# donglinb/ORB-SLAM-BIRDVIEW

Hardware: AMD Instinct MI355X
Metric: ORB features/sec per GPU (1280×720, 2000 kp, 8 levels) + Hamming matches/sec (higher is better)
Workload: dtype u8; 1 GPU; C3 1280x720 KITTI-style synthetic, 2000 features, 8 levels; width=1280, height=720, nfeatures=2000, nlevels=8, ini_th_fast=20, min_th_fast=7, batch_per_gpu=256, global_batch=256, parallelism=frame-sharded x1 (no collective), batches_in_flight=2

## Files before the change

### orb-slam-birdview_amd/csrc/extract_kernels.hip

```cpp
#include "glibc_trig.h"
#include "orbgpu_internal.h"
#include "pattern31_data.inc"

#include <algorithm>
#include <cstring>

namespace orbgpu {

__constant__ __attribute__((aligned(16))) int8_t c_pattern[1024] = {ORBGPU_PATTERN31_VALUES};
__constant__ __attribute__((aligned(16))) float c_pattern_f[1024] = {ORBGPU_PATTERN31_VALUES};

struct IcMaskTable {
    uint32_t m[64][4];
};
constexpr IcMaskTable make_ic_masks() {
    IcMaskTable t{};
    constexpr int umax[16] = {15, 15, 15, 15, 14, 14, 14, 13, 13, 12, 11, 10, 9, 8, 6, 3};
    for (int l = 0; l < 64; l++) {
        const int r = (l >> 1) < 30 ? (l >> 1) : 30, v = r - 15, h = l & 1;
        const int d = umax[v < 0 ? -v : v];
        for (int i = 0; i < 4; i++) {
            uint32_t m = 0;
            for (int j = 0; j < 4; j++) {
                const int u = 4 * (4 * h + i) + j;
                if (u >= 15 - d && u <= 15 + d) m |= 0xFFu << (8 * j);
            }
            t.m[l][i] = m;
        }
    }
    return t;
}
__constant__ __attribute__((aligned(16))) IcMaskTable c_ic_masks = make_ic_masks();

namespace {

struct LevelPtr {
    const uint8_t* p;
    int stride;
};

__device__ __forceinline__ LevelPtr level_ptr(const Geom* __restrict__ g, int l, const uint8_t* frames,
                                              long long framePitch, int rowStride, const uint8_t* pyr, int f) {
    if (l == 0) return {frames + (long long)f * framePitch, rowStride};
    return {pyr + (long long)f * g->pyr_bytes + g->L[l].pyr_off, g->L[l].pitch};
}

__device__ __forceinline__ void wave_lds_sync() {
    __builtin_amdgcn_fence(__ATOMIC_RELEASE, "wavefront");
    __builtin_amdgcn_wave_barrier();
    __builtin_amdgcn_fence(__ATOMIC_ACQUIRE, "wavefront");
}

__device__ __forceinline__ int lanes_below(unsigned long long mask) {
    return __builtin_amdgcn_mbcnt_hi((unsigned)(mask >> 32), __builtin_amdgcn_mbcnt_lo((unsigned)mask, 0));
}

}

typedef unsigned short ushort2_t __attribute__((ext_vector_type(2)));

__device__ __forceinline__ unsigned mul_hi_u24(unsigned a, unsigned b) {
    unsigned r;
    asm("v_mul_hi_u32_u24 %0, %1, %2" : "=v"(r) : "v"(a), "v"(b));
    return r;
}
typedef unsigned int uint32x4_t __attribute__((ext_vector_type(4)));

template <bool GENERIC>
__global__ __launch_bounds__(256) void k_resize(const Geom* __restrict__ g, const ResizeCoef* __restrict__ coef,
                                                int level, const uint8_t* __restrict__ frames, long long framePitch,
                                                int rowStride, uint8_t* __restrict__ pyr) {
    const int f = blockIdx.z;
    const int dw = g->L[level].w, dh = g->L[level].h;
    const int x0 = (blockIdx.x * 64 + (threadIdx.x & 63)) * 4;
    const int y = blockIdx.y * 4 + (threadIdx.x >> 6);
    if (x0 >= dw || y >= dh) return;
    const LevelPtr src = level_ptr(g, level - 1, frames, framePitch, rowStride, pyr, f);
    const ResizeCoef cy = coef[dw + y];
    const uint8_t* r0 = src.p + (long long)cy.s0 * src.stride;
    const uint8_t* r1 = src.p + (long long)cy.s1 * src.stride;
    uint32_t packed = 0;
#pragma unroll
    for (int i = 0; i < 4; i++) {
        const int x = min(x0 + i, dw - 1);
        const ResizeCoef cx = coef[x];
        const unsigned h0 = __umul24(r0[cx.s0], (unsigned)cx.c0) + __umul24(r0[cx.s1], (unsigned)cx.c1);
        const unsigned h1 = __umul24(r1[cx.s0], (unsigned)cx.c0) + __umul24(r1[cx.s1], (unsigned)cx.c1);
        const unsigned v =
            GENERIC ? min((__umul24((unsigned)cy.c0, h0) + __umul24((unsigned)cy.c1, h1) + (1u << 21)) >> 22, 255u)
                    : ((__umul24((unsigned)cy.c0, h0 >> 4) >> 16) + (__umul24((unsigned)cy.c1, h1 >> 4) >> 16) + 2) >> 2;
        packed |= (uint32_t)v << (8 * i);
    }
    uint8_t* dst = pyr + (long long)f * g->pyr_bytes + g->L[level].pyr_off;
    *reinterpret_cast<uint32_t*>(dst + (long long)y * g->L[level].pitch + x0) = packed;
}

template <bool GENERIC>
__device__ __forceinline__ int4 rs_row_entry(const ResizeCoef& c, int sy0) {
    return make_int4(__mul24(c.s0 - sy0, kRsPitch), __mul24(c.s1 - sy0, kRsPitch), GENERIC ? c.c0 : c.c0 << 12,
                     GENERIC ? c.c1 : c.c1 << 12);
}
template <bool GENERIC>
__device__ __forceinline__ unsigned rs_vpass(unsigned c0, unsigned c1, unsigned h0, unsigned h1) {
    if (GENERIC) return min((__umul24(c0, h0) + __umul24(c1, h1) + (1u << 21)) >> 22, 255u);
    return (mul_hi_u24(c0, h0 & ~15u) + mul_hi_u24(c1, h1 & ~15u) + 2) >> 2;
}

constexpr int kCpSc1 = 16;

__constant__ unsigned kRsMagic[18] = {0,    65536, 32768, 21846, 16384, 13108, 10923, 9363, 8192,
                                      7282, 6554,  5958,  5462,  5042,  4682,  4370,  4096, 3856};
template <int kRsTileH, bool GENERIC, int CP, int KP = 0>
__device__ __forceinline__ void resize_tile(const Geom* __restrict__ g, const ResizeCoef* __restrict__ coef, int level,
                                            const uint8_t* __restrict__ frames, long long framePitch, int rowStride,
                                            uint8_t* __restrict__ pyr, int f, int bx, int by, int tid, uint8_t* s_src,
                                            int4* s_cx, int4* s_cy, bool active) {
    constexpr int kRows = rs_rows(kRsTileH);
    constexpr int kQ = kRsPitch / 16;
    constexpr int kPer = KP > 0 ? KP : (kRows * kQ + 255) / 256;
    const int dw = g->L[level].w, dh = g->L[level].h;
    const int x0 = bx * kRsTileW, y0 = by * kRsTileH;
    const LevelPtr src = level_ptr(g, level - 1, frames, framePitch, rowStride, pyr, f);
    const int nx = min(kRsTileW, dw - x0), ny = min(kRsTileH, dh - y0);
    if (!active) {
        __syncthreads();
        return;
    }
    const bool vec16 = ((reinterpret_cast<uintptr_t>(src.p) | (uintptr_t)src.stride) & 15) == 0;
    const int sx0 = coef[x0].s0 & (vec16 ? ~15 : ~3), sx1 = coef[x0 + nx - 1].s1;
    const int sy0 = coef[dw + y0].s0, sy1 = coef[dw + y0 + ny - 1].s1;
    const int nr = sy1 - sy0 + 1;
    const uint8_t* base = src.p + (long long)sy0 * src.stride + sx0;
    int4 cxv = make_int4(0, 0, 0, 0), cyv = make_int4(0, 0, 0, 0);
    if (vec16) {
        const int nq = ((sx1 - sx0) >> 4) + 1;
        const unsigned magic = kRsMagic[nq];
        const int total = nr * nq;
        const uint64_t pb = reinterpret_cast<uint64_t>(base);
        const auto rsrc = __builtin_amdgcn_make_buffer_rsrc(reinterpret_cast<void*>(pb), 0, 0x7FFFFFFF, 0x00020000);
        uint4 v[kPer];
#pragma unroll
        for (int k = 0; k < kPer; k++) {
            const int i = min(tid + 256 * k, total - 1);
            const int r = (int)(__umul24((unsigned)i, magic) >> 16), q = i - (int)__umul24((unsigned)r, (unsigned)nq);
            const uint32x4_t w = __builtin_amdgcn_raw_buffer_load_b128(rsrc, (int)__umul24((unsigned)r, (unsigned)src.stride) + 16 * q, 0, CP);
            v[k] = make_uint4(w[0], w[1], w[2], w[3]);
        }
        if (tid < kRsTileW) {
            const ResizeCoef c = coef[x0 + min(tid, nx - 1)];
            cxv = make_int4(c.s0, c.s1, c.c0, c.c1);
        }
        if (tid < kRsTileH) {
            const ResizeCoef c = coef[dw + y0 + min(tid, ny - 1)];
            cyv = rs_row_entry<GENERIC>(c, sy0);
        }
#pragma unroll
        for (int k = 0; k < kPer; k++) {
            const int i = min(tid + 256 * k, total - 1);
            const int r = (int)(__umul24((unsigned)i, magic) >> 16), q = i - (int)__umul24((unsigned)r, (unsigned)nq);
            *reinterpret_cast<uint4*>(&s_src[r * kRsPitch + 16 * q]) = v[k];
        }
    } else {
        if (tid < kRsTileW) {
            const ResizeCoef c = coef[x0 + min(tid, nx - 1)];
            cxv = make_int4(c.s0, c.s1, c.c0, c.c1);
        }
        if (tid < kRsTileH) {
            const ResizeCoef c = coef[dw + y0 + min(tid, ny - 1)];
            cyv = rs_row_entry<GENERIC>(c, sy0);
        }
        if (((reinterpret_cast<uintptr_t>(src.p) | (uintptr_t)src.stride) & 3) == 0) {
            const int nw = (sx1 - sx0 + 4) >> 2;
            for (int i = tid; i < nr * 68; i += 256) {
                const int r = i / 68, wd = i - r * 68;
                if (wd < nw)
                    *reinterpret_cast<uint32_t*>(&s_src[r * kRsPitch + 4 * wd]) =
                        *reinterpret_cast<const uint32_t*>(base + (long long)r * src.stride + 4 * wd);
            }
        } else {
            const int nb = sx1 - sx0 + 1;
            for (int i = tid; i < nr * kRsPitch; i += 256) {
                const int r = i / kRsPitch, b = i - r * kRsPitch;
                if (b < nb) s_src[r * kRsPitch + b] = base[(long long)r * src.stride + b];
            }
        }
    }
    if (tid < kRsTileW) s_cx[tid] = cxv;
    if (tid < kRsTileH) s_cy[tid] = cyv;
// ... 2 lines not shown
    int o0[4], o1[4];
    unsigned c0[4], c1[4];
#pragma unroll
    for (int i = 0; i < 4; i++) {
        const int4 cx = s_cx[tx + i];
        o0[i] = cx.x - sx0;
        o1[i] = cx.y - sx0;
        c0[i] = cx.z;
        c1[i] = cx.w;
    }
    const uint64_t lb = reinterpret_cast<uint64_t>(pyr + (long long)f * g->pyr_bytes + g->L[level].pyr_off);
    const auto dsr = __builtin_amdgcn_make_buffer_rsrc(
        reinterpret_cast<void*>(((uint64_t)(uint32_t)__builtin_amdgcn_readfirstlane((unsigned)(lb >> 32)) << 32) |
                                (uint64_t)(uint32_t)__builtin_amdgcn_readfirstlane((unsigned)lb)),
        0, 0x7FFFFFFF, 0x00020000);
    const int pitch = g->L[level].pitch;
    const unsigned dcol = (unsigned)(x0 + tx);
    if (tx >= nx) return;
    const int bo = o0[0];
    const bool packed_ok = o1[3] - bo <= 7;
    if (__builtin_amdgcn_ballot_w64(!packed_ok) == 0) {
        unsigned sel[4];
        uint32_t cc[4];
#pragma unroll
        for (int i = 0; i < 4; i++) {
            sel[i] = (unsigned)(o0[i] - bo) | 0x0C00u | ((unsigned)(o1[i] - bo) << 16) | 0x0C000000u;
            cc[i] = c0[i] | (c1[i] << 16);
        }
        const int bw = bo >> 2, bsh = bo & 3;
#pragma unroll
        for (int pass = 0; pass < kRsTileH / 8; pass++) {
            const int ty = pass * 8 + (tid >> 5);
            if (ty >= ny) break;
            const int4 cy = s_cy[ty];
            const unsigned cy0 = (unsigned)cy.z, cy1 = (unsigned)cy.w;
            const uint32_t* q0 = reinterpret_cast<const uint32_t*>(&s_src[cy.x]) + bw;
            const uint32_t* q1 = reinterpret_cast<const uint32_t*>(&s_src[cy.y]) + bw;
            const uint32_t u0 = q0[0], u1 = q0[1], u2 = q0[2], w0 = q1[0], w1 = q1[1], w2 = q1[2];
            const uint32_t a0 = __builtin_amdgcn_alignbyte(u1, u0, bsh), a1 = __builtin_amdgcn_alignbyte(u2, u1, bsh);
            const uint32_t b0 = __builtin_amdgcn_alignbyte(w1, w0, bsh), b1 = __builtin_amdgcn_alignbyte(w2, w1, bsh);
            uint32_t packed = 0;
#pragma unroll
            for (int i = 0; i < 4; i++) {
                const unsigned h0 = __builtin_amdgcn_udot2(__builtin_bit_cast(ushort2_t, cc[i]),
                                                           __builtin_bit_cast(ushort2_t, __builtin_amdgcn_perm(a1, a0, sel[i])), 0u, false);
                const unsigned h1 = __builtin_amdgcn_udot2(__builtin_bit_cast(ushort2_t, cc[i]),
                                                           __builtin_bit_cast(ushort2_t, __builtin_amdgcn_perm(b1, b0, sel[i])), 0u, false);
                const unsigned v = rs_vpass<GENERIC>(cy0, cy1, h0, h1);
                packed |= v << (8 * i);
            }
            __builtin_amdgcn_raw_buffer_store_b32(packed, dsr, (int)(__umul24((unsigned)(y0 + ty), (unsigned)pitch) + dcol), 0, CP);
        }
        return;
    }
#pragma unroll
    for (int pass = 0; pass < kRsTileH / 8; pass++) {
        const int ty = pass * 8 + (tid >> 5);
        if (ty >= ny) break;
        const int4 cy = s_cy[ty];
        const uint8_t* r0 = &s_src[cy.x];
        const uint8_t* r1 = &s_src[cy.y];
        uint32_t packed = 0;
#pragma unroll
        for (int i = 0; i < 4; i++) {
            const unsigned h0 = __umul24(r0[o0[i]], c0[i]) + __umul24(r0[o1[i]], c1[i]);
            const unsigned h1 = __umul24(r1[o0[i]], c0[i]) + __umul24(r1[o1[i]], c1[i]);
            const unsigned v = rs_vpass<GENERIC>((unsigned)cy.z, (unsigned)cy.w, h0, h1);
            packed |= v << (8 * i);
        }
        __builtin_amdgcn_raw_buffer_store_b32(packed, dsr, (int)(__umul24((unsigned)(y0 + ty), (unsigned)pitch) + dcol), 0, CP);
    }
}

template <int kRsTileH, bool GENERIC, int KP>
__global__ __launch_bounds__(256) void k_resize_tiled(const Geom* __restrict__ g,
                                                      const ResizeCoef* __restrict__ coef, int level,
                                                      const uint8_t* __restrict__ frames, long long framePitch,
                                                      int rowStride, uint8_t* __restrict__ pyr) {
    extern __shared__ __attribute__((aligned(16))) uint8_t s_src[];
    __shared__ int4 s_cx[kRsTileW];
    __shared__ int4 s_cy[kRsTileH];
    resize_tile<kRsTileH, GENERIC, 0, KP>(g, coef, level, frames, framePitch, rowStride, pyr, blockIdx.z, blockIdx.x,
                                          blockIdx.y, threadIdx.x, s_src, s_cx, s_cy, true);
}

template <int CP>
__device__ __forceinline__ uint32_t chain_ld32(const uint8_t* p) {
    if constexpr (CP != 0)
        return __hip_atomic_load(reinterpret_cast<const uint32_t*>(p), __ATOMIC_RELAXED, __HIP_MEMORY_SCOPE_AGENT);
    else return *reinterpret_cast<const uint32_t*>(p);
}
template <int CP>
__device__ __forceinline__ uint32_t chain_ld8(const uint8_t* p) {
    if constexpr (CP != 0) {
        const uintptr_t a = reinterpret_cast<uintptr_t>(p);
        const uint32_t w = __hip_atomic_load(reinterpret_cast<const uint32_t*>(a & ~(uintptr_t)3), __ATOMIC_RELAXED,
                                             __HIP_MEMORY_SCOPE_AGENT);
        return (w >> (8 * (a & 3))) & 0xFFu;
    } else {
        return *p;
    }
}

template <bool GENERIC, int CP>
__device__ __forceinline__ void chain_job(const Geom* __restrict__ g, const ResizeCoef* __restrict__ coef,
                                          const ChainJob* __restrict__ J, const ChainSegment& sg, const RcoefOff& roff,
                                          const uint8_t* __restrict__ frames, long long framePitch, int rowStride,
                                          uint8_t* __restrict__ pyr, int f, int tid, uint8_t* sm, int4* sreg) {
    const int l = J->level, b = J->base;
    if (tid <= l) sreg[tid] = J->reg[tid];
    uint8_t* buf0 = sm;
    uint8_t* buf1 = sm + sg.buf_bytes;
    int4* sc = reinterpret_cast<int4*>(sm + 2 * sg.buf_bytes);
    uint8_t* fp = pyr + (long long)f * g->pyr_bytes;
    __syncthreads();
    {
        int e0 = 0;
        for (int k = b + 1; k <= l; k++) {
            const int4 R = sreg[k], S = sreg[k - 1];
            const int nx = R.y - R.x, ny = R.w - R.z;
            const int sp = (S.y - S.x + 3) & ~3;
            const ResizeCoef* cx = coef + roff.o[k];
            const int wk = g->L[k].w;
            for (int e = tid; e < nx + ny; e += 256) {
                int4 v;
                if (e < nx) {
                    const ResizeCoef c = cx[min(R.x + e, wk - 1)];
                    v = make_int4(c.s0 - S.x, c.s1 - S.x, c.c0, c.c1);
                } else {
                    const ResizeCoef c = cx[wk + R.z + (e - nx)];
                    v = rs_row_entry<GENERIC>(c, S.z);
                    v.x = (c.s0 - S.z) * sp;
                    v.y = (c.s1 - S.z) * sp;
                }
                sc[e0 + e] = v;
            }
            e0 += nx + ny;
        }
    }
    {
        const int4 R = sreg[b];
        const int p0 = (R.y - R.x + 3) & ~3, nq = p0 >> 2, ny = R.w - R.z, wb = g->L[b].w;
        const uint8_t* src = b == 0 ? frames + (long long)f * framePitch : fp + g->L[b].pyr_off;
        const int stride = b == 0 ? rowStride : g->L[b].pitch;
        const bool al = ((reinterpret_cast<uintptr_t>(src) | (uintptr_t)stride) & 3) == 0;
        const int QW = nq <= 16 ? 16 : nq <= 32 ? 32 : 64, RP = 256 / QW;
        for (int qb = 0; qb < nq; qb += QW)
            for (int r = tid / QW; r < ny; r += RP) {
                const int q = qb + (tid & (QW - 1));
                if (q >= nq) continue;
                const int col = R.x + 4 * q;
                const uint8_t* rp = src + (long long)(R.z + r) * stride;
                uint32_t v;
                if (al && col + 3 < wb) {
                    v = chain_ld32<CP>(rp + col);
                } else {
                    v = 0;
                    for (int t = 0; t < 4; t++)
                        if (col + t < wb) v |= chain_ld8<CP>(rp + col + t) << (8 * t);
                }
                *reinterpret_cast<uint32_t*>(buf0 + r * p0 + 4 * q) = v;
            }
    }
    __syncthreads();
    int e0 = 0;
    for (int k = b + 1; k <= l; k++) {
// ... 2085 lines not shown
            for (int l = 1; l < nl; l++)
                if (cseg[l] == sgi) lo = std::min(lo, l), hi = std::max(hi, l);
            for (int l = hi; l >= lo; l--) chainl(l);
            for (int l = hi; l >= lo; l--) {
                fast(l);
                octree(l);
            }
        }
    }
    for (int l = 0; l < nl; l++) {
        const int cap = g.L[l].kp_cap;
        for (int i = 0; i < cap; i += 16)
            for (int f = 0; f < nframes; f++)
                push(kFlowDescribe, l, f, -1, g.L[l].kp_base + i, std::min(16, cap - i), ctr(f, 2, 0), l + 1, 1);
    }
    constexpr int kLds = 160 * 1024 - 64;
    const int need = std::max({16 * g.fast_wave_bytes, 16 * kDescWaveBytes + 256, 4 * rsq, (int)octree_lds_bytes(g.node_cap)});
    if (need > kLds) return false;
    plan.ntasks = (int)tasks.size();
    plan.nframes = nframes;
    plan.nctr = kFlowCtrBase + 4 * nl * nframes;
    plan.lds_bytes = kLds;
    const long long room = kLds - (long long)octree_lds_bytes(g.node_cap);
    const long long want = ((long long)g.max_level_cand + 7) & ~7LL;
    plan.lds_keys = room > 0 ? (int)std::min(want, (room / 6) & ~7LL) : 0;
    plan.rs_quarter = rsq;
    plan.blocks = std::max(1, blocks);
    return true;
}

FlowArgs flow_args(const ExtractBuffers& b, const uint8_t* d_frames, long long frame_pitch, int row_stride, int nframes,
                   orb_keypoint* d_kps, uint8_t* d_desc, int* d_counts, int kp_cap) {
    FlowArgs A;
    std::memset(&A, 0, sizeof A);
    A.g = b.d_geom;
    A.rcoef = b.d_rcoef;
    std::memcpy(A.roff.o, b.rcoef_off, sizeof A.roff.o);
    A.cells = b.d_cells;
    A.frames = d_frames;
    A.framePitch = frame_pitch;
    A.rowStride = row_stride;
    A.pyr = b.d_pyr;
    A.cands = b.d_cands;
    A.candFirst = b.d_candFirst;
    A.keys = b.d_keys;
    A.knode = b.d_knode;
    A.lvlKps = b.d_lvlKps;
    A.lvlCount = b.d_lvlCount;
    A.err = b.d_err;
    A.errHost = b.err_host;
    A.outK = d_kps;
    A.outD = d_desc;
    A.outN = d_counts;
    A.kpCap = kp_cap;
    A.tasks = b.d_flow;
    A.ntasks = b.flow.ntasks;
    A.nframes = nframes;
    A.ctr = b.d_flow_ctr;
    A.ldsKeys = b.flow.lds_keys;
    A.rsQuarter = b.flow.rs_quarter;
    A.stamps = b.d_flow_stamps;
    A.chainJobs = b.d_chain;
    for (int i = 0; i < ORBGPU_MAX_LEVELS; i++) A.chainSeg[i] = b.flow_chain.seg[i];
    return A;
}

hipError_t launch_extract(const Geom& g, const ExtractBuffers& b, const uint8_t* d_frames, long long frame_pitch,
                          int row_stride, int nframes, orb_keypoint* d_kps, uint8_t* d_desc, int* d_counts,
                          int kp_cap, hipStream_t stream, KernelMarker marker, void* user) {
    if (nframes <= 0) return hipSuccess;
    if (b.d_flow && b.flow.nframes == nframes) {
        const bool fma = !(g.variant & ORB_VARIANT_NO_FMA);
        auto kern = g.fast_compact ? (fma ? k_extract_flow<48, true> : k_extract_flow<48, false>)
                                   : (fma ? k_extract_flow<kFastTilePitch, true> : k_extract_flow<kFastTilePitch, false>);
        if (marker) marker(user, ORB_K_FLOW, 1, stream);
        hipLaunchKernelGGL(kern, dim3(b.flow.blocks), dim3(kFlowThreads), (size_t)b.flow.lds_bytes, stream, b.d_flow_args);
        if (marker) marker(user, ORB_K_FLOW, 0, stream);
        return hipGetLastError();
    }
    auto resize = [&](int l, hipStream_t s) {
        const int t = g.L[l].rs_tiled;
        const ResizeCoef* cf = b.d_rcoef + b.rcoef_off[l];
        const bool gen = (g.variant & ORB_VARIANT_RESIZE_GENERIC) != 0;
        if (t & 3) {
            const int th = (t & 2) ? 32 : 16;
            const dim3 grid(cdiv(g.L[l].w, kRsTileW), cdiv(g.L[l].h, th), nframes);
            const size_t lds = (size_t)g.L[l].rs_span_rows * kRsPitch;
            const int kp = g.L[l].rs_chunks <= 512 ? 2 : g.L[l].rs_chunks <= 768 ? 3 : 0;
            auto kern = th == 32 ? (gen ? (kp == 2 ? k_resize_tiled<32, true, 2> : kp == 3 ? k_resize_tiled<32, true, 3>
                                                                                          : k_resize_tiled<32, true, 0>)
                                        : (kp == 2 ? k_resize_tiled<32, false, 2> : kp == 3 ? k_resize_tiled<32, false, 3>
                                                                                           : k_resize_tiled<32, false, 0>))
                                 : (gen ? (kp == 2 ? k_resize_tiled<16, true, 2> : k_resize_tiled<16, true, 0>)
                                        : (kp == 2 ? k_resize_tiled<16, false, 2> : k_resize_tiled<16, false, 0>));
            hipLaunchKernelGGL(kern, grid, dim3(256), lds, s, b.d_geom, cf, l, d_frames, frame_pitch, row_stride,
                               b.d_pyr);
        } else {
            hipLaunchKernelGGL(gen ? k_resize<true> : k_resize<false>, dim3(cdiv(g.L[l].w, 256), cdiv(g.L[l].h, 4), nframes),
                               dim3(256), 0, s, b.d_geom, cf, l, d_frames, frame_pitch, row_stride, b.d_pyr);
        }
    };
    auto fast = [&](int cbeg, int cnum, hipStream_t s, int* zero) {
        const int items = cnum * nframes;
        auto kern = g.fast_compact ? k_fast_wave<48> : k_fast_wave<kFastTilePitch>;
        const int ipw = nframes == 1 ? 1 : 2;
        hipLaunchKernelGGL(kern, dim3(cdiv(items, ipw)), dim3(64), (size_t)g.fast_wave_bytes, s, b.d_geom, b.d_cells,
                           d_frames, frame_pitch, row_stride, b.d_pyr, b.d_cands, b.d_candFirst, items, cbeg, cnum,
                           b.d_stamps, zero, ipw);
    };
    auto octree = [&](int lbase, int nl, hipStream_t s, int* err) {
        const bool one = nframes * nl <= 256;
        const int lk = one ? octree_lds_keys_whole_cu(g) : octree_lds_keys(g.node_cap);
        hipLaunchKernelGGL(k_octree<kOctreeThreads>, dim3(nframes, nl), dim3(kOctreeThreads),
                           octree_lds_bytes(g.node_cap) + (size_t)lk * 6, s, b.d_geom, b.d_cands, b.d_candFirst,
                           b.d_keys, b.d_knode, b.d_lvlKps, b.d_lvlCount, err, lk,
                           b.d_stamps ? b.d_stamps + (size_t)nframes * g.ncells * 8 : nullptr, lbase);
    };
    auto describe = [&](hipStream_t s) {
        unsigned long long* dst = b.d_stamps ? b.d_stamps + (size_t)nframes * (g.ncells * 8 + g.nlevels * 32) : nullptr;
        const int spw = nframes == 1 ? 1 : kDescSlotsPerWave;
        const unsigned gx = cdiv(g.nkpcap, kDescWaves * spw);
        hipLaunchKernelGGL((g.variant & ORB_VARIANT_NO_FMA) ? k_describe<false> : k_describe<true>, dim3(gx * nframes), dim3(64 * kDescWaves), 0, s, b.d_geom, d_frames, frame_pitch,
                           row_stride, b.d_pyr, b.d_lvlKps, b.d_lvlCount, d_kps, d_desc, d_counts, kp_cap, dst, spw,
                           b.d_err, b.err_host);
    };
    int* zero = b.zero_err ? b.d_err : nullptr;
    hipError_t fe = hipSuccess;
    const bool forked = b.fork_s2 != nullptr && g.nlevels > 1;
    const int c0 = g.L[1].cell_base;
    if (forked) {
        if ((fe = hipEventRecord(b.ev_fork, stream)) != hipSuccess || (fe = hipStreamWaitEvent(b.fork_s2, b.ev_fork, 0)) != hipSuccess)
            return fe;
        fast(0, c0, b.fork_s2, b.d_err + 1);
        octree(0, 1, b.fork_s2, b.d_err + 1);
        if ((fe = hipEventRecord(b.ev_join, b.fork_s2)) != hipSuccess) return fe;
    }
    if (marker) marker(user, ORB_K_RESIZE, 1, stream);
    if (b.chain.nseg && nframes <= kChainMaxFrames) {
        RcoefOff ro;
        std::memcpy(ro.o, b.rcoef_off, sizeof ro.o);
        const bool gen = (g.variant & ORB_VARIANT_RESIZE_GENERIC) != 0;
        for (int l = 1; l <= b.chain.first_base; l++) resize(l, stream);
        for (int sgi = 0; sgi < b.chain.nseg; sgi++) {
            const ChainSegment& sg = b.chain.seg[sgi];
            hipLaunchKernelGGL(gen ? k_pyramid_chain<true> : k_pyramid_chain<false>, dim3(sg.njobs, nframes), dim3(256),
                               (size_t)sg.lds_bytes, stream, b.d_geom, b.d_rcoef, b.d_chain, sg, ro, d_frames, frame_pitch,
                               row_stride, b.d_pyr);
        }
    } else {
        for (int l = 1; l < g.nlevels; l++) resize(l, stream);
    }
    if (marker) marker(user, ORB_K_RESIZE, 0, stream);
    if (marker) marker(user, ORB_K_FAST, 1, stream);
    if (forked) fast(c0, g.ncells - c0, stream, zero);
    else fast(0, g.ncells, stream, zero);
    if (marker) marker(user, ORB_K_FAST, 0, stream);
    if (marker) marker(user, ORB_K_OCTREE, 1, stream);
    if (forked) octree(1, g.nlevels - 1, stream, b.d_err);
    else octree(0, g.nlevels, stream, b.d_err);
    if (marker) marker(user, ORB_K_OCTREE, 0, stream);
    if (forked && (fe = hipStreamWaitEvent(stream, b.ev_join, 0)) != hipSuccess) return fe;
    if (marker) marker(user, ORB_K_DESCRIBE, 1, stream);
    describe(stream);
    if (marker) marker(user, ORB_K_DESCRIBE, 0, stream);
    return hipGetLastError();
}

// ... 2 lines not shown
```

### orb-slam-birdview_amd/csrc/orbgpu_abi.hip

```cpp
#include <algorithm>
#include <cmath>
#include <cstdio>
#include <cstdlib>
#include <cstring>
#include <new>
#include <string>
#include <vector>

#include "orbgpu_ctx.h"

namespace orbgpu {

thread_local std::string g_last_error;

void set_error(const char* what, hipError_t e) {
    char buf[512];
    if (e != hipSuccess) std::snprintf(buf, sizeof buf, "%s: %s", what, hipGetErrorString(e));
    else std::snprintf(buf, sizeof buf, "%s", what);
    g_last_error = buf;
}

static inline int round_half_even(float v) { return (int)std::nearbyint(v); }
static inline int round_half_even(double v) { return (int)std::nearbyint(v); }

// ... 53 lines not shown
        if (!vertical) {
            if (s0 < 0) { f = 0; s0 = 0; }
            if (s0 + 1 >= sw && s0 >= sw - 1) { f = 0; s0 = sw - 1; }
        }
        ResizeCoef rc;
        auto sat_short = [](int x) { return std::min(std::max(x, -32768), 32767); };
        rc.c0 = sat_short(round_half_even((1.f - f) * 2048));
        rc.c1 = sat_short(round_half_even(f * 2048));
        rc.s0 = std::min(std::max(s0, 0), sw - 1);
        rc.s1 = std::min(std::max(s0 + 1, 0), sw - 1);
        out.push_back(rc);
    }
}

int build_geometry(Ctx* c, int W, int H, Geom& g, std::vector<ResizeCoef>& coefs, int* rcoef_off) {
    std::memset(&g, 0, sizeof g);
    const int nl = c->p.nlevels;
    g.nlevels = nl;
    g.W = W;
    g.H = H;
    g.iniTh = std::min(std::max(c->p.iniThFAST, 0), 255);
    g.minTh = std::min(std::max(c->p.minThFAST, 0), 255);
    g.variant = c->p.variant;
    for (int i = 0; i < 16; i++) g.umax[i] = c->umax[i];
    for (int i = 0; i < 7; i++) g.gk[i] = c->gk[i];
    for (int sh = 0; sh < 4; sh++)
        for (int tc = 0; tc < kDescTapTiles; tc++)
            for (int l = 0; l < 64; l++) {
                uint8_t b[16];
                for (int e = 0; e < 16; e++) {
                    const int t = 16 * (l >> 4) + e - sh - (16 * tc + (l & 15));
                    b[e] = (uint8_t)(t >= 0 && t <= 6 ? c->gk[t] : 0);
                }
                std::memcpy(&g.desc_taps[(sh * kDescTapTiles + tc) * 64 + l], b, 16);
            }
    long long pyr = 0;
    int cells = 0, cand = 0, kpc = 0, maxN = 0, maxNini = 0, maxLevelCand = 0;
    coefs.clear();
    for (int l = 0; l < nl; l++) {
        LevelGeom& L = g.L[l];
        L.w = round_half_even((float)W * c->inv_scale[l]);
        L.h = round_half_even((float)H * c->inv_scale[l]);
        L.pitch = (L.w + 63) & ~63;
        if (l > 0) {
            L.pyr_off = pyr;
            pyr += (long long)L.pitch * L.h;
            rcoef_off[l] = (int)coefs.size();
            resize_coefs(g.L[l - 1].w, L.w, coefs, false);
            resize_coefs(g.L[l - 1].h, L.h, coefs, true);
            const ResizeCoef* cx = &coefs[rcoef_off[l]];
            const ResizeCoef* cy = cx + L.w;
            bool xfits = true;
            for (int x0 = 0; x0 < L.w && xfits; x0 += kRsTileW) {
                const int x1 = std::min(x0 + kRsTileW, L.w) - 1;
                xfits = cx[x1].s1 - (cx[x0].s0 & ~15) + 1 <= kRsPitch;
            }
            L.rs_tiled = 0;
            int span_rows[3] = {0, 0, 0};
            for (int i = 0; i < 3 && xfits; i++) {
                const int th = 16 << i;
                bool fits = true;
                for (int y0 = 0; y0 < L.h && fits; y0 += th) {
                    const int y1 = std::min(y0 + th, L.h) - 1;
                    span_rows[i] = std::max(span_rows[i], cy[y1].s1 - cy[y0].s0 + 1);
                    fits = cy[y1].s1 - cy[y0].s0 + 1 <= rs_rows(th);
                }
                if (fits) L.rs_tiled |= 1 << i;
            }
            L.rs_span_rows = (L.rs_tiled & 2) ? span_rows[1] : span_rows[0];
            L.rs_chunks = 0;
            if (L.rs_tiled & 3) {
                const int th = (L.rs_tiled & 2) ? 32 : 16;
                int nq_max = 0, nr_max = 0;
                for (int x0 = 0; x0 < L.w; x0 += kRsTileW) {
                    const int x1 = std::min(x0 + kRsTileW, L.w) - 1;
                    nq_max = std::max(nq_max, ((cx[x1].s1 - (cx[x0].s0 & ~15)) >> 4) + 1);
                }
                for (int y0 = 0; y0 < L.h; y0 += th) {
                    const int y1 = std::min(y0 + th, L.h) - 1;
                    nr_max = std::max(nr_max, cy[y1].s1 - cy[y0].s0 + 1);
                }
                L.rs_chunks = nq_max * nr_max;
            }
        }
        L.maxBX = L.w - kEdgeThreshold + 3;
        L.maxBY = L.h - kEdgeThreshold + 3;
        const float width = (float)(L.maxBX - kMinBorder), height = (float)(L.maxBY - kMinBorder);
        L.nCols = (int)(width / 30.f);
        L.nRows = (int)(height / 30.f);
        if (L.nCols <= 0 || L.nRows <= 0 || L.w < 2 || L.h < 2) return ORB_ERR_GEOMETRY;
        L.wCell = (int)std::ceil(width / L.nCols);
        L.hCell = (int)std::ceil(height / L.nRows);
        if (L.wCell + 6 > kFastMaxRoi || L.hCell + 6 > kFastMaxRoi) return ORB_ERR_GEOMETRY;
        L.cell_base = cells;
        cells += L.nCols * L.nRows;
        L.cell_cap = ((L.wCell + 1) / 2) * ((L.hCell + 1) / 2);
        L.cand_base = cand;
        L.cand_cap = L.cell_cap * L.nCols * L.nRows;
        cand += L.cand_cap;
        maxLevelCand = std::max(maxLevelCand, L.cand_cap);
        L.nfeat = c->n_per_level[l];
        L.nIni = (int)std::round(width / (float)(L.maxBY - kMinBorder));
        if (L.nIni <= 0) return ORB_ERR_GEOMETRY;
        L.hX = width / L.nIni;
        L.kp_cap = std::max(L.nfeat + 3, 4 * L.nIni) + 4;
        L.kp_base = kpc;
        kpc += L.kp_cap;
        maxN = std::max(maxN, L.nfeat);
        maxNini = std::max(maxNini, L.nIni);
        L.scale = c->scale[l];
        L.patch_size = (float)(int)(kPatchSize * c->scale[l]);
    }
    if (W > kMaxDim || H > kMaxDim) return ORB_ERR_GEOMETRY;
    g.ncells = cells;
    g.ncand = cand;
    g.nkpcap = kpc;
    g.pyr_bytes = (pyr + 255) & ~255LL;
    g.max_level_cand = maxLevelCand;
    int nc = std::max(maxN + 8, 4 * maxNini + 8);
    nc = (nc + 63) & ~63;
    g.node_cap = nc;
    fast_wave_layout(g);
    if (g.fast_wave_bytes > 64 * 1024 || octree_lds_bytes(nc) > 160 * 1024) return ORB_ERR_GEOMETRY;
    return ORB_OK;
}

template <class T>
static hipError_t grow(T*& p, size_t& cap, size_t need) {
    if (need <= cap && p) return hipSuccess;
    if (p) (void)hipFree(p);
    p = nullptr;
    cap = 0;
    hipError_t e = hipMalloc((void**)&p, std::max<size_t>(need, 256) * sizeof(T));
    if (e == hipSuccess) cap = std::max<size_t>(need, 256);
    return e;
}

static void build_chain(const Geom& g, const std::vector<ResizeCoef>& coefs, const int* off, std::vector<ChainJob>& jobs,
                        ChainPlan& plan, int first_base, int seg_len) {
    jobs.clear();
    plan = ChainPlan{};
    const int nl = g.nlevels;
    if (nl < 2 || first_base >= nl - 1) return;
    auto r4 = [](int x) { return (x + 3) & ~3; };
    for (int base = first_base; base < nl - 1; base += seg_len) {
        const int top = std::min(base + seg_len, nl - 1);
        ChainSegment sg;
        sg.job0 = (int)jobs.size();
        int bufb = 0, coefe = 0;
        for (int l = base + 1; l <= top; l++) {
            const int TW = l - base <= 2 ? 64 : 32, TH = l - base <= 2 ? 32 : 16;
            const int wl = g.L[l].w, hl = g.L[l].h;
            for (int y0 = 0; y0 < hl; y0 += TH)
                for (int x0 = 0; x0 < wl; x0 += TW) {
                    ChainJob J;
                    std::memset(&J, 0, sizeof J);
                    J.level = l;
                    J.base = base;
                    J.reg[l] = make_int4(x0, r4(std::min(x0 + TW, wl)), y0, std::min(y0 + TH, hl));
                    int ce = 0;
                    for (int k = l; k > base; k--) {
                        const int4 R = J.reg[k];
                        const ResizeCoef* cx = &coefs[off[k]];
                        const ResizeCoef* cy = cx + g.L[k].w;
                        const int sx0 = cx[R.x].s0, sx1 = cx[std::min(R.y, g.L[k].w) - 1].s1 + 1;
                        const int sy0 = cy[R.z].s0, sy1 = cy[R.w - 1].s1 + 1;
// ... 723 lines not shown
```

### orb-slam-birdview_amd/csrc/orbgpu_internal.h

```cpp
#pragma once
#include <hip/hip_runtime.h>
#include <stdint.h>

#include <vector>

#include "../../include/orbgpu.h"

namespace orbgpu {

constexpr int kEdgeThreshold = 19;
constexpr int kMinBorder = kEdgeThreshold - 3;
constexpr int kPatchSize = 31;
constexpr int kHalfPatch = 15;
constexpr int kMaxDim = 4096;
constexpr int kFastTilePitch = 80;
constexpr int kFastMaxRoi = 66;
constexpr int kOctreeThreads = 512;
constexpr int kCandRec = 8;
constexpr int kCandFirst = kCandRec - 1;
constexpr int kDescWin = 43;
constexpr int kDescWinPitch = 48;
constexpr int kDescBlur = 37;
constexpr int kDescBlurPitch = 40;
constexpr int kRtPitch = 44;
constexpr int kDescTapTiles = 3;
constexpr int kRsTileW = 128;
constexpr int kRsPitch = 272;
constexpr int rs_rows(int th) { return 2 * th + 8; }

struct LevelGeom {
    int w, h;
    int pitch;
    int rs_tiled;
    long long pyr_off;
    int maxBX, maxBY;
    int nCols, nRows, wCell, hCell;
    int cell_base;
    int cell_cap;
    int cand_base;
    int cand_cap;
    int nfeat;
    int kp_cap, kp_base;
    int nIni;
    float hX;
    float scale;
    float patch_size;
    int rs_span_rows;
    int rs_chunks;
};

struct Geom {
    int nlevels, W, H;
    int ncells;
    int ncand;
    int nkpcap;
    long long pyr_bytes;
    int iniTh, minTh;
    int variant;
    int node_cap;
    int max_level_cand;
    int fast_rows;
    int fast_drows;
    int fast_list;
    int fast_wave_bytes;
    int fast_compact;
    int umax[16];
    int gk[8];
    LevelGeom L[ORBGPU_MAX_LEVELS];
    int4 desc_taps[4 * kDescTapTiles * 64];
};

struct CellDesc {
    int lv;
    int iniX, iniY;
    int rwrh;
    int out_off;
    int xoyo;
    int pitch;
    int pyr_off;
    int roi;
    int m_nw;
    int runs;
    int m_runs;
    int pad[4];
};
__host__ __device__ inline uint32_t recip20(uint32_t n) { return ((1u << 20) + n - 1) / n; }

struct ResizeCoef {
    int s0, s1;
    int c0, c1;
};

struct ChainJob {
    int level, base, pad0, pad1;
    int4 reg[ORBGPU_MAX_LEVELS];
};
constexpr int kChainSeg = 4;
struct ChainSegment {
    int job0 = 0, njobs = 0;
    int buf_bytes = 0, coef_entries = 0, lds_bytes = 0;
};
struct ChainPlan {
    int nseg = 0;
    int first_base = 0;
    ChainSegment seg[ORBGPU_MAX_LEVELS];
};
constexpr int kSmallChainBase = 3;
constexpr int kChainMaxFrames = 2;
struct RcoefOff {
    int o[ORBGPU_MAX_LEVELS];
};

enum FlowKind : int { kFlowResize = 0, kFlowFast = 1, kFlowOctree = 2, kFlowDescribe = 3, kFlowChain = 4 };
struct FlowTask {
    int klf;
    int sig;
    int a, b;
    int dep, nd;
    int tgt;
    int seg;
};
struct FlowPlan {
    int ntasks = 0;
    int nframes = 0;
    int nctr = 0;
    int lds_bytes = 0;
    int lds_keys = 0;
    int rs_quarter = 0;
    int blocks = 0;
};
constexpr int kFlowCtrBase = 64;
constexpr int kFlowThreads = 1024;
constexpr int kFlowDefaultBlocks = 64;
bool build_flow(const Geom& g, int nframes, int blocks, const ChainPlan* chain, const std::vector<ChainJob>* jobs,
                std::vector<FlowTask>& tasks, FlowPlan& plan);

struct FlowArgs {
    const Geom* g;
    const ResizeCoef* rcoef;
    RcoefOff roff;
    const CellDesc* cells;
    const uint8_t* frames;
    long long framePitch;
    int rowStride;
    uint8_t* pyr;
    uint32_t* cands;
    uint32_t* candFirst;
    uint32_t* keys;
    uint16_t* knode;
    uint32_t* lvlKps;
    int* lvlCount;
    int* err;
    int* errHost;
    orb_keypoint* outK;
    uint8_t* outD;
    int* outN;
    int kpCap;
    const FlowTask* tasks;
    int ntasks;
    int nframes;
    int* ctr;
    int ldsKeys;
    int rsQuarter;
    unsigned long long* stamps;
    const ChainJob* chainJobs;
    ChainSegment chainSeg[ORBGPU_MAX_LEVELS];
};

struct ExtractBuffers {
    const Geom* d_geom;
    const ResizeCoef* d_rcoef;
    const CellDesc* d_cells;
    int rcoef_off[ORBGPU_MAX_LEVELS];
    const ChainJob* d_chain;
// ... 119 lines not shown
```

Before: 378.0 million features/s.

## Add row-strip resize kernel with dot2 horizontal pass for large batches

Adds a new pyramid resize kernel, k_resize_rows, used when the batch exceeds the chain frame limit and the source is 16-byte aligned. It uses 256x32 tiles with XCD-aware block remapping, b128 buffer loads into LDS, and per-wave 8-row strips. The horizontal pass uses udot2 on permuted bytes and reuses the previous row's horizontal result, and the vertical pass packs four pixels with perm. Host geometry computes the LDS rows and pitch and falls back to the old path when spans are too large. The cost is more code paths and inline asm, and the new path is only correct when the fit checks hold.

```diff
diff --git a/orb-slam-birdview_amd/csrc/extract_kernels.hip b/orb-slam-birdview_amd/csrc/extract_kernels.hip
--- a/orb-slam-birdview_amd/csrc/extract_kernels.hip
+++ b/orb-slam-birdview_amd/csrc/extract_kernels.hip
@@ -101,9 +101,35 @@
                      GENERIC ? c.c1 : c.c1 << 12);
 }
 template <bool GENERIC>
+__device__ __forceinline__ unsigned rs_hkeep(unsigned h) {
+    return GENERIC ? h : h & ~15u;
+}
+template <bool GENERIC>
+__device__ __forceinline__ unsigned rs_vsum(unsigned c0, unsigned c1, unsigned k0, unsigned k1) {
+    if (GENERIC) return min((__umul24(c0, k0) + __umul24(c1, k1) + (1u << 21)) >> 22, 255u);
+    return (mul_hi_u24(c0, k0) + mul_hi_u24(c1, k1) + 2) >> 2;
+}
+template <bool GENERIC>
 __device__ __forceinline__ unsigned rs_vpass(unsigned c0, unsigned c1, unsigned h0, unsigned h1) {
-    if (GENERIC) return min((__umul24(c0, h0) + __umul24(c1, h1) + (1u << 21)) >> 22, 255u);
-    return (mul_hi_u24(c0, h0 & ~15u) + mul_hi_u24(c1, h1 & ~15u) + 2) >> 2;
+    return rs_vsum<GENERIC>(c0, c1, rs_hkeep<GENERIC>(h0), rs_hkeep<GENERIC>(h1));
+}
+template <bool GENERIC>
+__device__ __forceinline__ uint32_t rs_vsum4(unsigned c0, unsigned c1, const unsigned (&k0)[4], const unsigned (&k1)[4]) {
+    if (GENERIC) {
+        uint32_t packed = 0;
+#pragma unroll
+        for (int i = 0; i < 4; i++) packed |= rs_vsum<true>(c0, c1, k0[i], k1[i]) << (8 * i);
+        return packed;
+    }
+    unsigned t[4];
+#pragma unroll
+    for (int i = 0; i < 4; i++) {
+        unsigned a, b;
+        asm("v_mul_hi_u32_u24 %0, %1, %2" : "=v"(a) : "s"(c0), "v"(k0[i]));
+        asm("v_mul_hi_u32_u24 %0, %1, %2" : "=v"(b) : "s"(c1), "v"(k1[i]));
+        t[i] = a + b + 2;
+    }
+    return __builtin_amdgcn_perm((t[2] | (t[3] << 16)) << 6, (t[0] | (t[1] << 16)) << 6, 0x07050301u);
 }
 
 constexpr int kCpSc1 = 16;
@@ -272,6 +298,84 @@
     __shared__ int4 s_cy[kRsTileH];
     resize_tile<kRsTileH, GENERIC, 0, KP>(g, coef, level, frames, framePitch, rowStride, pyr, blockIdx.z, blockIdx.x,
                                           blockIdx.y, threadIdx.x, s_src, s_cx, s_cy, true);
+}
+
+template <bool GENERIC, int KP>
+__global__ __launch_bounds__(256) void k_resize_rows(const Geom* __restrict__ g, const ResizeCoef* __restrict__ coef,
+                                                     int level, const uint8_t* __restrict__ frames,
+                                                     long long framePitch, int rowStride, uint8_t* __restrict__ pyr,
+                                                     int gx, unsigned gxRecip) {
+    extern __shared__ __attribute__((aligned(16))) uint8_t s_src[];
+    const int f = blockIdx.y;
+    const int nb = gridDim.x, bq = nb >> 3, br = nb & 7, xcd = blockIdx.x & 7, bj = blockIdx.x >> 3;
+    const int tile = (xcd < br ? xcd * (bq + 1) : br * (bq + 1) + (xcd - br) * bq) + bj;
+    const int by = (int)(((unsigned)tile * gxRecip) >> 20), bx = tile - by * gx;
+    const int tid = threadIdx.x;
+    const int wv = __builtin_amdgcn_readfirstlane(tid >> 6);
+    const int dw = g->L[level].w, dh = g->L[level].h, lp = g->L[level].rr_pitch;
+    const int x0 = bx * kRrTileW, y0 = by * kRrTileH;
+    const LevelPtr src = level_ptr(g, level - 1, frames, framePitch, rowStride, pyr, f);
+    const int nx = min(kRrTileW, dw - x0), ny = min(kRrTileH, dh - y0);
+    const ResizeCoef* __restrict__ cys = coef + dw;
+    const int sx0 = coef[x0].s0 & ~15, sx1 = coef[x0 + nx - 1].s1;
+    const int sy0 = cys[y0].s0, sy1 = cys[y0 + ny - 1].s1;
+    const int nr = sy1 - sy0 + 1, nq = ((sx1 - sx0) >> 4) + 1;
+    const uint64_t pb = reinterpret_cast<uint64_t>(src.p + (long long)sy0 * src.stride + sx0);
+    const auto rsrc = __builtin_amdgcn_make_buffer_rsrc(reinterpret_cast<void*>(pb), 0, (nr - 1) * src.stride + 16 * nq,
+                                                        0x00020000);
+    const int sq = tid & 31, sr = tid >> 5;
+    const int soff = sq < nq ? (int)__umul24((unsigned)sr, (unsigned)src.stride) + 16 * sq : 0x40000000;
+    uint32x4_t v[KP];
+#pragma unroll
+    for (int k = 0; k < KP; k++) v[k] = __builtin_amdgcn_raw_buffer_load_b128(rsrc, soff + 8 * k * src.stride, 0, 0);
+    const int tx = (tid & 63) * 4;
+    ResizeCoef cx[4];
+#pragma unroll
+    for (int i = 0; i < 4; i++) cx[i] = coef[min(x0 + tx + i, dw - 1)];
+    const int ys = y0 + wv * kRrStrip;
+    ResizeCoef cy[kRrStrip];
+#pragma unroll
+    for (int k = 0; k < kRrStrip; k++) cy[k] = cys[min(ys + k, dh - 1)];
+#pragma unroll
+    for (int k = 0; k < KP; k++)
+        if (sq < nq && sr + 8 * k < nr) *reinterpret_cast<uint32x4_t*>(&s_src[(sr + 8 * k) * lp + 16 * sq]) = v[k];
+    __syncthreads();
+    if (tx >= nx || ys >= y0 + ny) return;
+    const int bo = cx[0].s0 - sx0;
+    unsigned sel[4];
+    uint32_t cc[4];
+#pragma unroll
+    for (int i = 0; i < 4; i++) {
+        sel[i] = (unsigned)(cx[i].s0 - sx0 - bo) | 0x0C00u | ((unsigned)(cx[i].s1 - sx0 - bo) << 16) | 0x0C000000u;
+        cc[i] = (unsigned)cx[i].c0 | ((unsigned)cx[i].c1 << 16);
+    }
+    const uint8_t* lrow = s_src + (bo & ~3);
+    const unsigned bsh = bo & 3;
+    auto hpass = [&](unsigned (&h)[4], int srow) {
+        const uint32_t* q = reinterpret_cast<const uint32_t*>(lrow + (srow - sy0) * lp);
+        const uint32_t u0 = q[0], u1 = q[1], u2 = q[2];
+        const uint32_t a0 = __builtin_amdgcn_alignbyte(u1, u0, bsh), a1 = __builtin_amdgcn_alignbyte(u2, u1, bsh);
+#pragma unroll
+        for (int i = 0; i < 4; i++)
+            h[i] = rs_hkeep<GENERIC>(__builtin_amdgcn_udot2(__builtin_bit_cast(ushort2_t, cc[i]),
+                                                            __builtin_bit_cast(ushort2_t, __builtin_amdgcn_perm(a1, a0, sel[i])), 0u, false));
+    };
+    const uint64_t lb = reinterpret_cast<uint64_t>(pyr + (long long)f * g->pyr_bytes + g->L[level].pyr_off);
+    const auto dsr = __builtin_amdgcn_make_buffer_rsrc(reinterpret_cast<void*>(lb), 0, 0x7FFFFFFF, 0x00020000);
+    const int pitch = g->L[level].pitch;
+    unsigned hc[4] = {0, 0, 0, 0}, hn[4];
+    int cur = -1;
+#pragma unroll
+    for (int k = 0; k < kRrStrip; k++) {
+        if (ys + k >= y0 + ny) break;
+        if (cy[k].s0 != cur) hpass(hc, cy[k].s0);
+        hpass(hn, cy[k].s1);
+        const unsigned c0 = GENERIC ? cy[k].c0 : cy[k].c0 << 12, c1 = GENERIC ? cy[k].c1 : cy[k].c1 << 12;
+        __builtin_amdgcn_raw_buffer_store_b32(rs_vsum4<GENERIC>(c0, c1, hc, hn), dsr, tx, (ys + k) * pitch + x0, 0);
+#pragma unroll
+        for (int i = 0; i < 4; i++) hc[i] = hn[i];
+        cur = cy[k].s1;
+    }
 }
 
 template <int CP>
@@ -2523,7 +2627,16 @@
         const int t = g.L[l].rs_tiled;
         const ResizeCoef* cf = b.d_rcoef + b.rcoef_off[l];
         const bool gen = (g.variant & ORB_VARIANT_RESIZE_GENERIC) != 0;
-        if (t & 3) {
+        const bool src16 = l > 1 || ((reinterpret_cast<uintptr_t>(d_frames) | (uintptr_t)frame_pitch | (uintptr_t)row_stride) & 15) == 0;
+        if (nframes > kChainMaxFrames && g.L[l].rr_rows > 0 && src16) {
+            const int gx = cdiv(g.L[l].w, kRrTileW), gy = cdiv(g.L[l].h, kRrTileH);
+            const size_t lds = (size_t)g.L[l].rr_rows * g.L[l].rr_pitch;
+            const bool kp6 = g.L[l].rr_rows <= 48;
+            auto kern = gen ? (kp6 ? k_resize_rows<true, 6> : k_resize_rows<true, kRrMaxRows / 8>)
+                            : (kp6 ? k_resize_rows<false, 6> : k_resize_rows<false, kRrMaxRows / 8>);
+            hipLaunchKernelGGL(kern, dim3(gx * gy, nframes), dim3(256), lds, s, b.d_geom, cf, l, d_frames, frame_pitch,
+                               row_stride, b.d_pyr, gx, recip20((uint32_t)gx));
+        } else if (t & 3) {
             const int th = (t & 2) ? 32 : 16;
             const dim3 grid(cdiv(g.L[l].w, kRsTileW), cdiv(g.L[l].h, th), nframes);
             const size_t lds = (size_t)g.L[l].rs_span_rows * kRsPitch;
diff --git a/orb-slam-birdview_amd/csrc/orbgpu_abi.hip b/orb-slam-birdview_amd/csrc/orbgpu_abi.hip
--- a/orb-slam-birdview_amd/csrc/orbgpu_abi.hip
+++ b/orb-slam-birdview_amd/csrc/orbgpu_abi.hip
@@ -159,6 +159,9 @@
                 }
                 L.rs_chunks = nq_max * nr_max;
             }
+            const RrGeom rr = rr_geometry(cx, L.w, cy, L.h);
+            L.rr_rows = rr.rows;
+            L.rr_pitch = rr.pitch;
         }
         L.maxBX = L.w - kEdgeThreshold + 3;
         L.maxBY = L.h - kEdgeThreshold + 3;
diff --git a/orb-slam-birdview_amd/csrc/orbgpu_internal.h b/orb-slam-birdview_amd/csrc/orbgpu_internal.h
--- a/orb-slam-birdview_amd/csrc/orbgpu_internal.h
+++ b/orb-slam-birdview_amd/csrc/orbgpu_internal.h
@@ -27,6 +27,11 @@
 constexpr int kRsTileW = 128;
 constexpr int kRsPitch = 272;
 constexpr int rs_rows(int th) { return 2 * th + 8; }
+constexpr int kRrTileW = 256;
+constexpr int kRrTileH = 32;
+constexpr int kRrStrip = 8;
+constexpr int kRrMaxRows = 64;
+constexpr int kRrMaxChunks = 32;
 
 struct LevelGeom {
     int w, h;
@@ -47,6 +52,8 @@
     float patch_size;
     int rs_span_rows;
     int rs_chunks;
+    int rr_rows;
+    int rr_pitch;
 };
 
 struct Geom {
@@ -90,6 +97,28 @@
     int s0, s1;
     int c0, c1;
 };
+
+struct RrGeom {
+    int rows, pitch;
+};
+inline RrGeom rr_geometry(const ResizeCoef* cx, int w, const ResizeCoef* cy, int h) {
+    const RrGeom none{0, 0};
+    for (int x = 0; x < w; x += 4)
+        if (cx[x + 3 < w ? x + 3 : w - 1].s1 - cx[x].s0 > 7) return none;
+    int span = 0, rows = 0;
+    for (int x0 = 0; x0 < w; x0 += kRrTileW) {
+        const int x1 = (x0 + kRrTileW < w ? x0 + kRrTileW : w) - 1;
+        const int s = cx[x1].s1 - (cx[x0].s0 & ~15) + 1;
+        span = s > span ? s : span;
+    }
+    for (int y0 = 0; y0 < h; y0 += kRrTileH) {
+        const int y1 = (y0 + kRrTileH < h ? y0 + kRrTileH : h) - 1;
+        const int r = cy[y1].s1 - cy[y0].s0 + 1;
+        rows = r > rows ? r : rows;
+    }
+    if ((span + 15) / 16 > kRrMaxChunks || rows > kRrMaxRows) return none;
+    return RrGeom{rows, (span + 11 + 15) & ~15};
+}
 
 struct ChainJob {
     int level, base, pad0, pad1;
```

Measured after the change: 386.3 million features/s, median of 6. +2.2%, better.
